# gsalzer/mythril

Hardware: AMD Instinct MI355X
Metric: constraint-candidate evals/sec + % z3 queries discharged on-GPU (higher is better)
Workload: dtype u32 (256-bit as 8x32-bit limbs)

## Files before the change

mythril_amd/csrc/u256.h:

```cpp
#pragma once
#include <math.h>
#include <stdint.h>

#define PF_INL __device__ __forceinline__

#include "u256_cols.h"

namespace pf {

struct u256 {
    uint32_t l[8];
};

PF_INL u256 zero256() {
    u256 r;
#pragma unroll
    for (int i = 0; i < 8; i++) r.l[i] = 0;
    return r;
}

PF_INL u256 ones256() {
    u256 r;
#pragma unroll
    for (int i = 0; i < 8; i++) r.l[i] = 0xffffffffu;
    return r;
}

PF_INL u256 add256(const u256& a, const u256& b) {
    u256 r;
    uint32_t c = 0;
#pragma unroll
    for (int i = 0; i < 8; i++) {
        uint32_t co;
        r.l[i] = __builtin_addc(a.l[i], b.l[i], c, &co);
        c = co;
    }
    return r;
}

PF_INL u256 add256c(const u256& a, const u256& b, uint32_t* cout) {
    u256 r;
    uint32_t c = 0;
#pragma unroll
    for (int i = 0; i < 8; i++) {
        uint32_t co;
        r.l[i] = __builtin_addc(a.l[i], b.l[i], c, &co);
        c = co;
    }
    *cout = c;
    return r;
}

PF_INL u256 sub256(const u256& a, const u256& b) {
    u256 r;
    uint32_t c = 0;
#pragma unroll
    for (int i = 0; i < 8; i++) {
        uint32_t co;
        r.l[i] = __builtin_subc(a.l[i], b.l[i], c, &co);
        c = co;
    }
    return r;
}

PF_INL u256 sub256b(const u256& a, const u256& b, uint32_t* bout) {
    u256 r;
    uint32_t c = 0;
#pragma unroll
    for (int i = 0; i < 8; i++) {
        uint32_t co;
        r.l[i] = __builtin_subc(a.l[i], b.l[i], c, &co);
        c = co;
    }
    *bout = c;
    return r;
}

PF_INL uint32_t ult256(const u256& a, const u256& b) {
    uint32_t c = 0;
#pragma unroll
    for (int i = 0; i < 8; i++) {
        uint32_t co;
        (void)__builtin_subc(a.l[i], b.l[i], c, &co);
        c = co;
    }
    return c;
}

PF_INL uint32_t eq256(const u256& a, const u256& b) {
    uint32_t d = 0;
#pragma unroll
    for (int i = 0; i < 8; i++) d |= a.l[i] ^ b.l[i];
    return d == 0;
}

PF_INL uint32_t iszero256(const u256& a) {
    uint32_t d = 0;
#pragma unroll
    for (int i = 0; i < 8; i++) d |= a.l[i];
    return d == 0;
}

PF_INL u256 neg256(const u256& a) { return sub256(zero256(), a); }

PF_INL u256 not256(const u256& a) {
    u256 r;
#pragma unroll
    for (int i = 0; i < 8; i++) r.l[i] = ~a.l[i];
    return r;
}

PF_INL uint32_t lane_mask(uint32_t c) {
    uint32_t m = 0u - (uint32_t)(c != 0u);
#ifndef PF_HOST_MAC
    asm volatile("" : "+v"(m));
#endif
    return m;
}

PF_INL u256 sel256(uint32_t c, const u256& a, const u256& b) {
    const uint32_t m = lane_mask(c);
    u256 r;
#pragma unroll
    for (int i = 0; i < 8; i++) r.l[i] = (a.l[i] & m) | (b.l[i] & ~m);
    return r;
}

#ifndef PF_HOST_MAC
PF_INL uint32_t wave_max_u32(uint32_t v) {
#pragma unroll
    for (int o = 32; o >= 1; o >>= 1) v = max(v, (uint32_t)__shfl_xor((int)v, o));
    return __builtin_amdgcn_readfirstlane(v);
}
PF_INL bool wave_any(bool p) { return __ballot(p) != 0ull; }
PF_INL uint32_t umulhi32(uint32_t a, uint32_t b) { return __umulhi(a, b); }
#else
PF_INL uint32_t wave_max_u32(uint32_t v) { return v; }
PF_INL bool wave_any(bool p) { return p; }
PF_INL uint32_t umulhi32(uint32_t a, uint32_t b) { return (uint32_t)(((uint64_t)a * b) >> 32); }
#endif

#define PF_COL_NEXT(k)                                   \
    r.l[k] = (uint32_t)acc;                              \
    acc = (acc >> 32) | ((uint64_t)hi << 32);            \
    hi = 0u;

PF_INL u256 mul256(const u256& a, const u256& b) {
    const uint32_t *x = a.l, *y = b.l;
    u256 r;
    uint64_t acc = 0;
    uint32_t hi = 0;
    col64_1(acc, x[0], y[0]);
    PF_COL_NEXT(0)
    col96_2(acc, hi, x[0], x[1], y[1], y[0]);
    PF_COL_NEXT(1)
    col96_3(acc, hi, x[0], x[1], x[2], y[2], y[1], y[0]);
    PF_COL_NEXT(2)
    col96_4(acc, hi, x[0], x[1], x[2], x[3], y[3], y[2], y[1], y[0]);
    PF_COL_NEXT(3)
    col96_5(acc, hi, x[0], x[1], x[2], x[3], x[4], y[4], y[3], y[2], y[1], y[0]);
    PF_COL_NEXT(4)
    col96_6(acc, hi, x[0], x[1], x[2], x[3], x[4], x[5], y[5], y[4], y[3], y[2], y[1], y[0]);
    PF_COL_NEXT(5)
    col64_7(acc, x[0], x[1], x[2], x[3], x[4], x[5], x[6], y[6], y[5], y[4], y[3], y[2], y[1], y[0]);
    r.l[6] = (uint32_t)acc;
    acc >>= 32;
    col64_8(acc, x[0], x[1], x[2], x[3], x[4], x[5], x[6], x[7], y[7], y[6], y[5], y[4], y[3], y[2], y[1], y[0]);
    r.l[7] = (uint32_t)acc;
    return r;
}

PF_INL u256 sqr256(const u256& a) {
    const uint32_t* x = a.l;
    u256 r;
    r.l[0] = 0u;
    uint64_t acc = 0;
    uint32_t hi = 0;
    col64_1(acc, x[0], x[1]);
    PF_COL_NEXT(1)
    col96_1(acc, hi, x[0], x[2]);
    PF_COL_NEXT(2)
    col96_2(acc, hi, x[0], x[1], x[3], x[2]);
    PF_COL_NEXT(3)
    col96_2(acc, hi, x[0], x[1], x[4], x[3]);
    PF_COL_NEXT(4)
    col96_3(acc, hi, x[0], x[1], x[2], x[5], x[4], x[3]);
    PF_COL_NEXT(5)
    col64_3(acc, x[0], x[1], x[2], x[6], x[5], x[4]);
    r.l[6] = (uint32_t)acc;
    acc >>= 32;
    col64_4(acc, x[0], x[1], x[2], x[3], x[7], x[6], x[5], x[4]);
    r.l[7] = (uint32_t)acc;
    u256 c;
#pragma unroll
    for (int i = 7; i >= 1; i--) c.l[i] = (r.l[i] << 1) | (r.l[i - 1] >> 31);
    c.l[0] = 0u;
    u256 d;
#pragma unroll
    for (int i = 0; i < 4; i++) {
        uint64_t q = 0;
        col64_1(q, x[i], x[i]);
        d.l[2 * i] = (uint32_t)q;
        d.l[2 * i + 1] = (uint32_t)(q >> 32);
    }
    return add256(c, d);
}
#undef PF_COL_NEXT

PF_INL uint32_t mul256_overflows(const u256& a, const u256& b) {
    uint32_t hi = 0;
    u256 r = zero256();
#pragma unroll
    for (int i = 0; i < 8; i++) {
        uint64_t carry = 0;
#pragma unroll
        for (int j = 0; j < 8; j++) {
            if (i + j < 8) {
                uint64_t t = (uint64_t)a.l[i] * b.l[j] + r.l[i + j] + carry;
                r.l[i + j] = (uint32_t)t;
                carry = t >> 32;
            } else {
                hi |= (a.l[i] != 0u && b.l[j] != 0u) ? 1u : 0u;
            }
        }
        hi |= (carry != 0) ? 1u : 0u;
    }
    return hi;
}

PF_INL u256 shl256(const u256& a, uint32_t s, uint32_t big) {
    u256 x = a;
    if (__builtin_expect(1, 1)) {
        uint32_t m = (s >> 7) & 1;
#pragma unroll
        for (int i = 7; i >= 0; i--) x.l[i] = m ? (i >= 4 ? x.l[i - 4] : 0u) : x.l[i];
        m = (s >> 6) & 1;
#pragma unroll
        for (int i = 7; i >= 0; i--) x.l[i] = m ? (i >= 2 ? x.l[i - 2] : 0u) : x.l[i];
        m = (s >> 5) & 1;
#pragma unroll
        for (int i = 7; i >= 0; i--) x.l[i] = m ? (i >= 1 ? x.l[i - 1] : 0u) : x.l[i];
    }
    uint32_t bs = s & 31;
    u256 r;
#pragma unroll
    for (int i = 7; i >= 1; i--) r.l[i] = bs ? ((x.l[i] << bs) | (x.l[i - 1] >> (32 - bs))) : x.l[i];
    r.l[0] = x.l[0] << bs;
    return sel256(big, zero256(), r);
}

PF_INL u256 shr256(const u256& a, uint32_t s, uint32_t f) {
    u256 x = a;
    uint32_t m = (s >> 7) & 1;
#pragma unroll
    for (int i = 0; i < 8; i++) x.l[i] = m ? (i + 4 < 8 ? x.l[i + 4] : f) : x.l[i];
    m = (s >> 6) & 1;
#pragma unroll
    for (int i = 0; i < 8; i++) x.l[i] = m ? (i + 2 < 8 ? x.l[i + 2] : f) : x.l[i];
    m = (s >> 5) & 1;
#pragma unroll
    for (int i = 0; i < 8; i++) x.l[i] = m ? (i + 1 < 8 ? x.l[i + 1] : f) : x.l[i];
    uint32_t bs = s & 31;
    u256 r;
#pragma unroll
    for (int i = 0; i < 7; i++) r.l[i] = bs ? ((x.l[i] >> bs) | (x.l[i + 1] << (32 - bs))) : x.l[i];
    r.l[7] = bs ? ((x.l[7] >> bs) | (f << (32 - bs))) : x.l[7];
    return r;
}

PF_INL uint32_t clz256(const u256& a) {
    uint32_t n = 0, done = 0;
#pragma unroll
    for (int i = 7; i >= 0; i--) {
        uint32_t z = a.l[i] ? (uint32_t)__builtin_clz(a.l[i]) : 32u;
        n += done ? 0u : z;
        done |= (a.l[i] != 0u);
    }
    return n;
}

PF_INL double rcp_f64(double x) {
#ifndef PF_HOST_MAC
    double r = __builtin_amdgcn_rcp(x);
    double e = fma(-x, r, 1.0);
    r = fma(r, e, r);
    e = fma(-x, r, 1.0);
    return fma(r, e, r);
#else
    return 1.0 / x;
#endif
}

// ... 94 lines not shown
#pragma unroll
        for (int i = 0; i + j <= 8; i++) {
            const uint64_t p = (uint64_t)q * (i < 8 ? b.l[i] : 0u) + carry;
            carry = p >> 32;
            uint32_t bo;
            u[j + i] = __builtin_subc(u[j + i], (uint32_t)p, borrow, &bo);
            borrow = bo;
        }
        if (wave_any(borrow != 0u)) {
            const uint32_t m = 0u - borrow;
            q -= borrow;
            uint32_t c = 0;
#pragma unroll
            for (int i = 0; i + j <= 8; i++) {
                uint32_t co;
                u[j + i] = __builtin_addc(u[j + i], (i < 8 ? b.l[i] : 0u) & m, c, &co);
                c = co;
            }
        }
        Q.l[j] = q;
    }
    u256 R;
#pragma unroll
    for (int i = 0; i < 8; i++) R.l[i] = u[i];
    *q = sel256(bz, ones256(), Q);
    *r = sel256(bz, a, R);
}

PF_INL void tbl_put(uint2* tbl, uint32_t stride, uint32_t j, const u256& v) {
#pragma unroll
    for (int p = 0; p < 4; p++) tbl[(j * 4u + p) * stride] = make_uint2(v.l[2 * p], v.l[2 * p + 1]);
}
PF_INL u256 tbl_get(const uint2* tbl, uint32_t stride, uint32_t j) {
    u256 v;
#pragma unroll
    for (int p = 0; p < 4; p++) {
        const uint2 q = tbl[(j * 4u + p) * stride];
        v.l[2 * p] = q.x;
        v.l[2 * p + 1] = q.y;
    }
    return v;
}

template <int WB = 3>
PF_INL u256 exp256(const u256& base, const u256& e, uint32_t nbits, uint2* tbl, uint32_t stride) {
    static_assert(WB >= 1 && WB <= 3, "window");
    constexpr uint32_t NT = 1u << WB;
    u256 r = zero256();
    r.l[0] = 1u;
    if (nbits == 0u) return r;
    tbl_put(tbl, stride, 0u, r);
    tbl_put(tbl, stride, 1u, base);
    if constexpr (WB == 2) {
        const u256 b2 = sqr256(base);
        tbl_put(tbl, stride, 2u, b2);
        tbl_put(tbl, stride, 3u, mul256(b2, base));
    } else {
#pragma unroll 1
        for (uint32_t j = 2; j < NT; j++) {
            const u256 f = tbl_get(tbl, stride, (j & 1u) ? j - 1u : j >> 1);
            const u256 g = (j & 1u) ? base : f;
            tbl_put(tbl, stride, j, mul256(f, g));
        }
    }
    const uint32_t nd = (nbits + WB - 1u) / WB;
    const uint32_t rest = WB * (nd - 1u);
    r = tbl_get(tbl, stride, shr256(e, rest, 0u).l[0] & (NT - 1u));
    u256 ex = shl256(e, (256u - rest) & 255u, 0u);
#pragma unroll 1
    for (uint32_t i = 1; i < nd; i++) {
#pragma unroll 1
        for (int k = 0; k < WB; k++) r = sqr256(r);
        const uint32_t d = ex.l[7] >> (32 - WB);
#pragma unroll
        for (int k = 7; k >= 1; k--) ex.l[k] = (ex.l[k] << WB) | (ex.l[k - 1] >> (32 - WB));
        ex.l[0] <<= WB;
        r = mul256(r, tbl_get(tbl, stride, d));
    }
    return r;
}

template <int WB = 2>
PF_INL u256 exp256_w32(const u256& base, uint32_t e, uint32_t nbits, uint2* tbl, uint32_t stride) {
    static_assert(WB == 2, "window");
    u256 one = zero256();
    one.l[0] = 1u;
    tbl_put(tbl, stride, 1u, base);
    const u256 b2 = sqr256(base);
    tbl_put(tbl, stride, 2u, b2);
    tbl_put(tbl, stride, 3u, mul256(b2, base));
    if (nbits == 0u) return one;
    const uint32_t nd = (nbits + WB - 1u) / WB;
    uint32_t d = (e >> (WB * (nd - 1u))) & 3u;
    u256 r = sel256((uint32_t)(d == 0u), one, tbl_get(tbl, stride, d));
#pragma unroll 1
    for (uint32_t i = nd - 1u; i-- > 0u;) {
#pragma unroll 1
        for (int k = 0; k < WB; k++) r = sqr256(r);
        d = (e >> (WB * i)) & 3u;
        r = mul256(r, sel256((uint32_t)(d == 0u), one, tbl_get(tbl, stride, d)));
    }
    return r;
}

#ifndef PF_EXP_SPLIT
#define PF_EXP_SPLIT 8
#endif
#define PF_EXP_WINDOW (PF_EXP_SPLIT <= 20 ? 2 : 3)
#define PF_EXP_TBL_ENTRIES (1 << PF_EXP_WINDOW)

PF_INL uint32_t funnel(uint32_t hi, uint32_t lo, uint32_t s) {
    return (uint32_t)((((uint64_t)hi << 32) | lo) >> s);
}

template <int L>
PF_INL void tsqr(const uint32_t* a, uint32_t* out) {
    uint32_t r[L];
#pragma unroll
    for (int i = 0; i < L; i++) r[i] = 0u;
#pragma unroll
    for (int i = 0; 2 * i + 1 < L; i++) {
        uint64_t c = 0;
#pragma unroll
        for (int j = i + 1; i + j < L; j++) {
            c = (uint64_t)a[i] * a[j] + (uint64_t)r[i + j] + (c >> 32);
            r[i + j] = (uint32_t)c;
        }
    }
#pragma unroll
    for (int i = L - 1; i >= 1; i--) r[i] = funnel(r[i], r[i - 1], 31u);
    r[0] <<= 1;
    uint32_t d[L];
#pragma unroll
    for (int i = 0; 2 * i < L; i++) {
        const uint64_t q = (uint64_t)a[i] * a[i];
        d[2 * i] = (uint32_t)q;
        if (2 * i + 1 < L) d[2 * i + 1] = (uint32_t)(q >> 32);
    }
    uint32_t c = 0;
#pragma unroll
    for (int i = 0; i < L; i++) {
        uint32_t co;
        out[i] = __builtin_addc(r[i], d[i], c, &co);
        c = co;
    }
}

template <int TL, uint32_t TM, int Q>
PF_INL void t_steps(uint32_t* t, uint32_t k0, uint32_t k1) {
    constexpr int L = TL - Q;
#pragma unroll 1
    for (uint32_t k = k0; k < k1; k++) {
        uint32_t sq[L];
        tsqr<L>(t, sq);
        const uint32_t sh = 32u - (k + 1u - 32u * Q);
        uint32_t c = 0;
#pragma unroll
        for (int i = Q; i < TL; i++) {
            const uint32_t lo = i > Q ? sq[i > Q ? i - Q - 1 : 0] : 0u;
            uint32_t co;
            t[i] = __builtin_addc(t[i], funnel(sq[i - Q], lo, sh), c, &co);
            c = co;
        }
        t[TL - 1] &= TM;
    }
}


PF_INL u256 div_odd_small(const u256& a, uint32_t o, uint32_t inv) {
    u256 q;
    uint32_t s = 0;
#pragma unroll
    for (int i = 0; i < 8; i++) {
        const uint32_t ai = a.l[i] - s;
        const uint32_t bo = a.l[i] < s;
        q.l[i] = ai * inv;
        s = umulhi32(q.l[i], o) + bo;
    }
    return q;
}

constexpr int v2c(int i) { return (i & 1) ? 0 : 1 + v2c(i >> 1); }
constexpr int v2fact(int j) { return j <= 1 ? 0 : v2c(j) + v2fact(j - 1); }
constexpr int exp_terms(int m) {
    int j = 1;
    while ((j + 1) * (m + 2) - v2fact(j + 1) < 256) j++;
    return j;
}
constexpr uint32_t inv32(uint32_t o) {
    uint32_t x = o;
    for (int i = 0; i < 5; i++) x *= 2u - o * x;
    return x;
}
constexpr int prefix_val(int m, int i) { return (i - 1) * (m + 2) - v2fact(i - 1); }

template <int L>
PF_INL u256 tmul(const u256& a, const u256& b) {
    if constexpr (L >= 8) {
        return mul256(a, b);
    } else {
        u256 r = zero256();
#pragma unroll
        for (int i = 0; i < L; i++) {
            uint64_t c = 0;
#pragma unroll
            for (int j = 0; i + j < L; j++) {
                c = (uint64_t)a.l[i] * b.l[j] + (uint64_t)r.l[i + j] + (c >> 32);
                r.l[i + j] = (uint32_t)c;
            }
        }
        return r;
    }
}

template <int L>
PF_INL u256 sub_mul_small(const u256& a, const u256& b, uint32_t c) {
    u256 r = zero256();
    uint32_t carry = 0, bw = 0;
#pragma unroll
    for (int i = 0; i < L; i++) {
        const uint64_t p = (uint64_t)b.l[i] * c + carry;
        carry = (uint32_t)(p >> 32);
        uint32_t bo;
        r.l[i] = __builtin_subc(a.l[i], (uint32_t)p, bw, &bo);
        bw = bo;
    }
    return r;
}

template <int L>
PF_INL u256 div_odd_small(const u256& a, uint32_t o, uint32_t inv) {
    u256 q = zero256();
    uint32_t s = 0;
#pragma unroll
    for (int i = 0; i < L; i++) {
        const uint32_t ai = a.l[i] - s;
        const uint32_t bo = a.l[i] < s;
        q.l[i] = ai * inv;
        s = umulhi32(q.l[i], o) + bo;
    }
    return q;
}

template <int S, int L>
PF_INL u256 shl_const(const u256& a) {
    constexpr int LS = S / 32, BS = S % 32;
    u256 r = zero256();
#pragma unroll
    for (int i = LS; i < L; i++) {
        const uint32_t hi = a.l[i - LS];
        const uint32_t lo = i - LS - 1 >= 0 ? a.l[i - LS - 1 >= 0 ? i - LS - 1 : 0] : 0u;
        r.l[i] = BS ? funnel(hi, lo, 32 - BS) : hi;
    }
    return r;
}

template <int M, int I, int J>
PF_INL u256 horner(const u256& nt, const u256& tt) {
    constexpr int S = M + 2 - v2c(I);
    constexpr int P = 256 - prefix_val(M, I);
    constexpr int L = (P + 31) / 32;
    constexpr int LG = (P - S + 31) / 32;
    constexpr int O = I >> v2c(I);
    u256 inner = zero256();
    if constexpr (I < J) inner = horner<M, I + 1, J>(nt, tt);
    u256 g = I > 1 ? sub_mul_small<LG>(nt, tt, (uint32_t)(I - 1)) : nt;
    if (O > 1) g = div_odd_small<LG>(g, (uint32_t)O, inv32((uint32_t)O));
    u256 h = shl_const<S, L>(g);
    if constexpr (I < J) h = tmul<L>(h, inner);
    h.l[0] += 1u;
    return h;
}

PF_INL u256 exp256_split(const u256& base, const u256& e, uint2* tbl, uint32_t stride,
                         uint64_t* pt = nullptr) {
#if defined(PF_PROFILE_UNITS) && !defined(PF_HOST_MAC)
#define PF_EXP_STAMP(k)                                        \
    if (pt) {                                                  \
        const uint64_t t_ = __builtin_amdgcn_s_memtime();      \
        pt[k] += t_ - t_last;                                  \
        t_last = t_;                                           \
    }
    uint64_t t_last = __builtin_amdgcn_s_memtime();
#else
#define PF_EXP_STAMP(k)
    (void)pt;
#endif
    constexpr int M = PF_EXP_SPLIT;
    static_assert(M >= 8 && M <= 84, "split");
    constexpr int T = 254 - M;
    constexpr int TL = (T + 31) / 32;
    constexpr uint32_t TM = (T % 32) ? ((1u << (T % 32)) - 1u) : 0xffffffffu;
    constexpr int TB = (T + 3 + 31) / 32;
    constexpr int J = exp_terms(M);
    constexpr int WB = PF_EXP_WINDOW;
    const uint32_t odd = base.l[0] & 1u;
    const uint32_t e_big =
        (e.l[0] >= 256u) | ((e.l[1] | e.l[2] | e.l[3] | e.l[4] | e.l[5] | e.l[6] | e.l[7]) != 0u);
    u256 e0;
#pragma unroll
    for (int i = 0; i < 8; i++)
        e0.l[i] = 32 * i + 32 <= M ? e.l[i] : (32 * i < M ? e.l[i] & ((1u << (M % 32)) - 1u) : 0u);
    const uint32_t nb0 = wave_max_u32(256u - clz256(e0));
    u256 r;
    if constexpr (M <= 32 && WB == 2)
        r = exp256_w32<WB>(base, e0.l[0], nb0 < (uint32_t)M ? nb0 : (uint32_t)M, tbl, stride);
    else
        r = exp256<WB>(base, e0, nb0 < (uint32_t)M ? nb0 : (uint32_t)M, tbl, stride);
    PF_EXP_STAMP(0)
    u256 n = shr256(e, (uint32_t)M, 0u);
#pragma unroll
    for (int i = 0; i < 8; i++) n.l[i] = i < TL - 1 ? n.l[i] : (i == TL - 1 ? n.l[i] & TM : 0u);
    if (wave_any(odd & (iszero256(n) ^ 1u))) {
        tbl_put(tbl, stride, 1u, r);
        uint32_t t[TL];
        {
            uint32_t sq[TB];
            if constexpr (M <= 32 && WB == 2 && TB == 8) {
                const u256 b2 = tbl_get(tbl, stride, 2u);
#pragma unroll
                for (int i = 0; i < TB; i++) sq[i] = b2.l[i];
            } else {
                tsqr<TB>(base.l, sq);
            }
            sq[0] -= 1u;
#pragma unroll
            for (int i = 0; i < TL; i++) t[i] = funnel(i + 1 < TB ? sq[i + 1 < TB ? i + 1 : 0] : 0u, sq[i], 3u);
            t[TL - 1] &= TM;
        }
        t_steps<TL, TM, 0>(t, 1u, M < 32 ? (uint32_t)M : 32u);
        if (M > 32) t_steps<TL, TM, 1>(t, 32u, M < 64 ? (uint32_t)M : 64u);
        if (M > 64) t_steps<TL, TM, 2>(t, 64u, (uint32_t)M);
        u256 tt = zero256();
#pragma unroll
        for (int i = 0; i < TL; i++) tt.l[i] = t[i];
        PF_EXP_STAMP(1)
        const u256 nt = tmul<(256 - (M + 2) + 31) / 32>(n, tt);
        u256 h = horner<M, 1, J>(nt, tt);
        u256 one = zero256();
        one.l[0] = 1u;
        h = sel256(odd, h, one);
        r = mul256(tbl_get(tbl, stride, 1u), h);
        PF_EXP_STAMP(2)
    }
    return sel256((odd ^ 1u) & e_big, zero256(), r);
#undef PF_EXP_STAMP
}

}
```

mythril_amd/csrc/u256_cols.h:

```cpp
#pragma once
namespace pf {
#ifndef PF_HOST_MAC

PF_INL void col96_1(uint64_t& acc, uint32_t& hi, uint32_t x0, uint32_t y0) {
    uint64_t p0;
    asm("v_mad_u64_u32 %[acc], %[p0], %[x0], %[y0], %[acc]\n\ts_nop 1\n\tv_addc_co_u32_e64 %[hi], %[p0], %[hi], 0, %[p0]"
        : [acc] "+v"(acc), [hi] "+v"(hi), [p0] "=&s"(p0)
        : [x0] "v"(x0), [y0] "v"(y0));
}

PF_INL void col96_2(uint64_t& acc, uint32_t& hi, uint32_t x0, uint32_t x1, uint32_t y0, uint32_t y1) {
    uint64_t p0; uint64_t p1;
    asm("v_mad_u64_u32 %[acc], %[p0], %[x0], %[y0], %[acc]\n\tv_mad_u64_u32 %[acc], %[p1], %[x1], %[y1], %[acc]\n\ts_nop 0\n\tv_addc_co_u32_e64 %[hi], %[p0], %[hi], 0, %[p0]\n\tv_addc_co_u32_e64 %[hi], %[p1], %[hi], 0, %[p1]"
        : [acc] "+v"(acc), [hi] "+v"(hi), [p0] "=&s"(p0), [p1] "=&s"(p1)
        : [x0] "v"(x0), [x1] "v"(x1), [y0] "v"(y0), [y1] "v"(y1));
}

PF_INL void col96_3(uint64_t& acc, uint32_t& hi, uint32_t x0, uint32_t x1, uint32_t x2, uint32_t y0, uint32_t y1, uint32_t y2) {
    uint64_t p0; uint64_t p1; uint64_t p2;
    asm("v_mad_u64_u32 %[acc], %[p0], %[x0], %[y0], %[acc]\n\tv_mad_u64_u32 %[acc], %[p1], %[x1], %[y1], %[acc]\n\tv_mad_u64_u32 %[acc], %[p2], %[x2], %[y2], %[acc]\n\tv_addc_co_u32_e64 %[hi], %[p0], %[hi], 0, %[p0]\n\tv_addc_co_u32_e64 %[hi], %[p1], %[hi], 0, %[p1]\n\tv_addc_co_u32_e64 %[hi], %[p2], %[hi], 0, %[p2]"
        : [acc] "+v"(acc), [hi] "+v"(hi), [p0] "=&s"(p0), [p1] "=&s"(p1), [p2] "=&s"(p2)
        : [x0] "v"(x0), [x1] "v"(x1), [x2] "v"(x2), [y0] "v"(y0), [y1] "v"(y1), [y2] "v"(y2));
}

// ... 26 lines not shown
}

PF_INL void col64_2(uint64_t& acc, uint32_t x0, uint32_t x1, uint32_t y0, uint32_t y1) {
    uint64_t p;
    asm("v_mad_u64_u32 %[acc], %[p], %[x0], %[y0], %[acc]\n\tv_mad_u64_u32 %[acc], %[p], %[x1], %[y1], %[acc]"
        : [acc] "+v"(acc), [p] "=&s"(p)
        : [x0] "v"(x0), [x1] "v"(x1), [y0] "v"(y0), [y1] "v"(y1));
}

PF_INL void col64_3(uint64_t& acc, uint32_t x0, uint32_t x1, uint32_t x2, uint32_t y0, uint32_t y1, uint32_t y2) {
    uint64_t p;
    asm("v_mad_u64_u32 %[acc], %[p], %[x0], %[y0], %[acc]\n\tv_mad_u64_u32 %[acc], %[p], %[x1], %[y1], %[acc]\n\tv_mad_u64_u32 %[acc], %[p], %[x2], %[y2], %[acc]"
        : [acc] "+v"(acc), [p] "=&s"(p)
        : [x0] "v"(x0), [x1] "v"(x1), [x2] "v"(x2), [y0] "v"(y0), [y1] "v"(y1), [y2] "v"(y2));
}

PF_INL void col64_4(uint64_t& acc, uint32_t x0, uint32_t x1, uint32_t x2, uint32_t x3, uint32_t y0, uint32_t y1, uint32_t y2, uint32_t y3) {
    uint64_t p;
    asm("v_mad_u64_u32 %[acc], %[p], %[x0], %[y0], %[acc]\n\tv_mad_u64_u32 %[acc], %[p], %[x1], %[y1], %[acc]\n\tv_mad_u64_u32 %[acc], %[p], %[x2], %[y2], %[acc]\n\tv_mad_u64_u32 %[acc], %[p], %[x3], %[y3], %[acc]"
        : [acc] "+v"(acc), [p] "=&s"(p)
        : [x0] "v"(x0), [x1] "v"(x1), [x2] "v"(x2), [x3] "v"(x3), [y0] "v"(y0), [y1] "v"(y1), [y2] "v"(y2), [y3] "v"(y3));
}

PF_INL void col64_5(uint64_t& acc, uint32_t x0, uint32_t x1, uint32_t x2, uint32_t x3, uint32_t x4, uint32_t y0, uint32_t y1, uint32_t y2, uint32_t y3, uint32_t y4) {
    uint64_t p;
    asm("v_mad_u64_u32 %[acc], %[p], %[x0], %[y0], %[acc]\n\tv_mad_u64_u32 %[acc], %[p], %[x1], %[y1], %[acc]\n\tv_mad_u64_u32 %[acc], %[p], %[x2], %[y2], %[acc]\n\tv_mad_u64_u32 %[acc], %[p], %[x3], %[y3], %[acc]\n\tv_mad_u64_u32 %[acc], %[p], %[x4], %[y4], %[acc]"
        : [acc] "+v"(acc), [p] "=&s"(p)
        : [x0] "v"(x0), [x1] "v"(x1), [x2] "v"(x2), [x3] "v"(x3), [x4] "v"(x4), [y0] "v"(y0), [y1] "v"(y1), [y2] "v"(y2), [y3] "v"(y3), [y4] "v"(y4));
}

PF_INL void col64_6(uint64_t& acc, uint32_t x0, uint32_t x1, uint32_t x2, uint32_t x3, uint32_t x4, uint32_t x5, uint32_t y0, uint32_t y1, uint32_t y2, uint32_t y3, uint32_t y4, uint32_t y5) {
    uint64_t p;
    asm("v_mad_u64_u32 %[acc], %[p], %[x0], %[y0], %[acc]\n\tv_mad_u64_u32 %[acc], %[p], %[x1], %[y1], %[acc]\n\tv_mad_u64_u32 %[acc], %[p], %[x2], %[y2], %[acc]\n\tv_mad_u64_u32 %[acc], %[p], %[x3], %[y3], %[acc]\n\tv_mad_u64_u32 %[acc], %[p], %[x4], %[y4], %[acc]\n\tv_mad_u64_u32 %[acc], %[p], %[x5], %[y5], %[acc]"
        : [acc] "+v"(acc), [p] "=&s"(p)
        : [x0] "v"(x0), [x1] "v"(x1), [x2] "v"(x2), [x3] "v"(x3), [x4] "v"(x4), [x5] "v"(x5), [y0] "v"(y0), [y1] "v"(y1), [y2] "v"(y2), [y3] "v"(y3), [y4] "v"(y4), [y5] "v"(y5));
}

PF_INL void col64_7(uint64_t& acc, uint32_t x0, uint32_t x1, uint32_t x2, uint32_t x3, uint32_t x4, uint32_t x5, uint32_t x6, uint32_t y0, uint32_t y1, uint32_t y2, uint32_t y3, uint32_t y4, uint32_t y5, uint32_t y6) {
    uint64_t p;
    asm("v_mad_u64_u32 %[acc], %[p], %[x0], %[y0], %[acc]\n\tv_mad_u64_u32 %[acc], %[p], %[x1], %[y1], %[acc]\n\tv_mad_u64_u32 %[acc], %[p], %[x2], %[y2], %[acc]\n\tv_mad_u64_u32 %[acc], %[p], %[x3], %[y3], %[acc]\n\tv_mad_u64_u32 %[acc], %[p], %[x4], %[y4], %[acc]\n\tv_mad_u64_u32 %[acc], %[p], %[x5], %[y5], %[acc]\n\tv_mad_u64_u32 %[acc], %[p], %[x6], %[y6], %[acc]"
        : [acc] "+v"(acc), [p] "=&s"(p)
        : [x0] "v"(x0), [x1] "v"(x1), [x2] "v"(x2), [x3] "v"(x3), [x4] "v"(x4), [x5] "v"(x5), [x6] "v"(x6), [y0] "v"(y0), [y1] "v"(y1), [y2] "v"(y2), [y3] "v"(y3), [y4] "v"(y4), [y5] "v"(y5), [y6] "v"(y6));
}

PF_INL void col64_8(uint64_t& acc, uint32_t x0, uint32_t x1, uint32_t x2, uint32_t x3, uint32_t x4, uint32_t x5, uint32_t x6, uint32_t x7, uint32_t y0, uint32_t y1, uint32_t y2, uint32_t y3, uint32_t y4, uint32_t y5, uint32_t y6, uint32_t y7) {
    uint64_t p;
    asm("v_mad_u64_u32 %[acc], %[p], %[x0], %[y0], %[acc]\n\tv_mad_u64_u32 %[acc], %[p], %[x1], %[y1], %[acc]\n\tv_mad_u64_u32 %[acc], %[p], %[x2], %[y2], %[acc]\n\tv_mad_u64_u32 %[acc], %[p], %[x3], %[y3], %[acc]\n\tv_mad_u64_u32 %[acc], %[p], %[x4], %[y4], %[acc]\n\tv_mad_u64_u32 %[acc], %[p], %[x5], %[y5], %[acc]\n\tv_mad_u64_u32 %[acc], %[p], %[x6], %[y6], %[acc]\n\tv_mad_u64_u32 %[acc], %[p], %[x7], %[y7], %[acc]"
        : [acc] "+v"(acc), [p] "=&s"(p)
        : [x0] "v"(x0), [x1] "v"(x1), [x2] "v"(x2), [x3] "v"(x3), [x4] "v"(x4), [x5] "v"(x5), [x6] "v"(x6), [x7] "v"(x7), [y0] "v"(y0), [y1] "v"(y1), [y2] "v"(y2), [y3] "v"(y3), [y4] "v"(y4), [y5] "v"(y5), [y6] "v"(y6), [y7] "v"(y7));
}

#else

PF_INL void col96_1(uint64_t& acc, uint32_t& hi, uint32_t x0, uint32_t y0) {
    { unsigned __int128 t = (unsigned __int128)x0 * y0 + acc; acc = (uint64_t)t; hi += (uint32_t)(t >> 64); }
}

PF_INL void col96_2(uint64_t& acc, uint32_t& hi, uint32_t x0, uint32_t x1, uint32_t y0, uint32_t y1) {
    { unsigned __int128 t = (unsigned __int128)x0 * y0 + acc; acc = (uint64_t)t; hi += (uint32_t)(t >> 64); }
    { unsigned __int128 t = (unsigned __int128)x1 * y1 + acc; acc = (uint64_t)t; hi += (uint32_t)(t >> 64); }
}

PF_INL void col96_3(uint64_t& acc, uint32_t& hi, uint32_t x0, uint32_t x1, uint32_t x2, uint32_t y0, uint32_t y1, uint32_t y2) {
    { unsigned __int128 t = (unsigned __int128)x0 * y0 + acc; acc = (uint64_t)t; hi += (uint32_t)(t >> 64); }
    { unsigned __int128 t = (unsigned __int128)x1 * y1 + acc; acc = (uint64_t)t; hi += (uint32_t)(t >> 64); }
    { unsigned __int128 t = (unsigned __int128)x2 * y2 + acc; acc = (uint64_t)t; hi += (uint32_t)(t >> 64); }
}

PF_INL void col96_4(uint64_t& acc, uint32_t& hi, uint32_t x0, uint32_t x1, uint32_t x2, uint32_t x3, uint32_t y0, uint32_t y1, uint32_t y2, uint32_t y3) {
    { unsigned __int128 t = (unsigned __int128)x0 * y0 + acc; acc = (uint64_t)t; hi += (uint32_t)(t >> 64); }
    { unsigned __int128 t = (unsigned __int128)x1 * y1 + acc; acc = (uint64_t)t; hi += (uint32_t)(t >> 64); }
    { unsigned __int128 t = (unsigned __int128)x2 * y2 + acc; acc = (uint64_t)t; hi += (uint32_t)(t >> 64); }
    { unsigned __int128 t = (unsigned __int128)x3 * y3 + acc; acc = (uint64_t)t; hi += (uint32_t)(t >> 64); }
}

PF_INL void col96_5(uint64_t& acc, uint32_t& hi, uint32_t x0, uint32_t x1, uint32_t x2, uint32_t x3, uint32_t x4, uint32_t y0, uint32_t y1, uint32_t y2, uint32_t y3, uint32_t y4) {
    { unsigned __int128 t = (unsigned __int128)x0 * y0 + acc; acc = (uint64_t)t; hi += (uint32_t)(t >> 64); }
    { unsigned __int128 t = (unsigned __int128)x1 * y1 + acc; acc = (uint64_t)t; hi += (uint32_t)(t >> 64); }
    { unsigned __int128 t = (unsigned __int128)x2 * y2 + acc; acc = (uint64_t)t; hi += (uint32_t)(t >> 64); }
    { unsigned __int128 t = (unsigned __int128)x3 * y3 + acc; acc = (uint64_t)t; hi += (uint32_t)(t >> 64); }
    { unsigned __int128 t = (unsigned __int128)x4 * y4 + acc; acc = (uint64_t)t; hi += (uint32_t)(t >> 64); }
}

PF_INL void col96_6(uint64_t& acc, uint32_t& hi, uint32_t x0, uint32_t x1, uint32_t x2, uint32_t x3, uint32_t x4, uint32_t x5, uint32_t y0, uint32_t y1, uint32_t y2, uint32_t y3, uint32_t y4, uint32_t y5) {
    { unsigned __int128 t = (unsigned __int128)x0 * y0 + acc; acc = (uint64_t)t; hi += (uint32_t)(t >> 64); }
    { unsigned __int128 t = (unsigned __int128)x1 * y1 + acc; acc = (uint64_t)t; hi += (uint32_t)(t >> 64); }
    { unsigned __int128 t = (unsigned __int128)x2 * y2 + acc; acc = (uint64_t)t; hi += (uint32_t)(t >> 64); }
    { unsigned __int128 t = (unsigned __int128)x3 * y3 + acc; acc = (uint64_t)t; hi += (uint32_t)(t >> 64); }
    { unsigned __int128 t = (unsigned __int128)x4 * y4 + acc; acc = (uint64_t)t; hi += (uint32_t)(t >> 64); }
    { unsigned __int128 t = (unsigned __int128)x5 * y5 + acc; acc = (uint64_t)t; hi += (uint32_t)(t >> 64); }
}

PF_INL void col64_1(uint64_t& acc, uint32_t x0, uint32_t y0) {
    acc += (uint64_t)x0 * y0;
}

PF_INL void col64_2(uint64_t& acc, uint32_t x0, uint32_t x1, uint32_t y0, uint32_t y1) {
    acc += (uint64_t)x0 * y0;
    acc += (uint64_t)x1 * y1;
}

PF_INL void col64_3(uint64_t& acc, uint32_t x0, uint32_t x1, uint32_t x2, uint32_t y0, uint32_t y1, uint32_t y2) {
    acc += (uint64_t)x0 * y0;
    acc += (uint64_t)x1 * y1;
    acc += (uint64_t)x2 * y2;
}

PF_INL void col64_4(uint64_t& acc, uint32_t x0, uint32_t x1, uint32_t x2, uint32_t x3, uint32_t y0, uint32_t y1, uint32_t y2, uint32_t y3) {
    acc += (uint64_t)x0 * y0;
    acc += (uint64_t)x1 * y1;
    acc += (uint64_t)x2 * y2;
    acc += (uint64_t)x3 * y3;
}

PF_INL void col64_5(uint64_t& acc, uint32_t x0, uint32_t x1, uint32_t x2, uint32_t x3, uint32_t x4, uint32_t y0, uint32_t y1, uint32_t y2, uint32_t y3, uint32_t y4) {
    acc += (uint64_t)x0 * y0;
    acc += (uint64_t)x1 * y1;
    acc += (uint64_t)x2 * y2;
    acc += (uint64_t)x3 * y3;
    acc += (uint64_t)x4 * y4;
}

PF_INL void col64_6(uint64_t& acc, uint32_t x0, uint32_t x1, uint32_t x2, uint32_t x3, uint32_t x4, uint32_t x5, uint32_t y0, uint32_t y1, uint32_t y2, uint32_t y3, uint32_t y4, uint32_t y5) {
    acc += (uint64_t)x0 * y0;
    acc += (uint64_t)x1 * y1;
    acc += (uint64_t)x2 * y2;
    acc += (uint64_t)x3 * y3;
    acc += (uint64_t)x4 * y4;
    acc += (uint64_t)x5 * y5;
}

PF_INL void col64_7(uint64_t& acc, uint32_t x0, uint32_t x1, uint32_t x2, uint32_t x3, uint32_t x4, uint32_t x5, uint32_t x6, uint32_t y0, uint32_t y1, uint32_t y2, uint32_t y3, uint32_t y4, uint32_t y5, uint32_t y6) {
    acc += (uint64_t)x0 * y0;
    acc += (uint64_t)x1 * y1;
    acc += (uint64_t)x2 * y2;
    acc += (uint64_t)x3 * y3;
    acc += (uint64_t)x4 * y4;
    acc += (uint64_t)x5 * y5;
    acc += (uint64_t)x6 * y6;
}

PF_INL void col64_8(uint64_t& acc, uint32_t x0, uint32_t x1, uint32_t x2, uint32_t x3, uint32_t x4, uint32_t x5, uint32_t x6, uint32_t x7, uint32_t y0, uint32_t y1, uint32_t y2, uint32_t y3, uint32_t y4, uint32_t y5, uint32_t y6, uint32_t y7) {
    acc += (uint64_t)x0 * y0;
    acc += (uint64_t)x1 * y1;
    acc += (uint64_t)x2 * y2;
    acc += (uint64_t)x3 * y3;
    acc += (uint64_t)x4 * y4;
    acc += (uint64_t)x5 * y5;
    acc += (uint64_t)x6 * y6;
    acc += (uint64_t)x7 * y7;
}

#endif
}
```

Baseline: 6.786 billion.

## Reformulate exp Horner with precomputed constant addends, drop per-term odd divisions

```diff
diff --git a/mythril_amd/csrc/u256.h b/mythril_amd/csrc/u256.h
--- a/mythril_amd/csrc/u256.h
+++ b/mythril_amd/csrc/u256.h
@@ -133,11 +133,9 @@
     return __builtin_amdgcn_readfirstlane(v);
 }
 PF_INL bool wave_any(bool p) { return __ballot(p) != 0ull; }
-PF_INL uint32_t umulhi32(uint32_t a, uint32_t b) { return __umulhi(a, b); }
 #else
 PF_INL uint32_t wave_max_u32(uint32_t v) { return v; }
 PF_INL bool wave_any(bool p) { return p; }
-PF_INL uint32_t umulhi32(uint32_t a, uint32_t b) { return (uint32_t)(((uint64_t)a * b) >> 32); }
 #endif
 
 #define PF_COL_NEXT(k)                                   \
@@ -538,7 +536,16 @@
 #pragma unroll 1
     for (uint32_t k = k0; k < k1; k++) {
         uint32_t sq[L];
-        tsqr<L>(t, sq);
+        if constexpr (L == 8) {
+            u256 a;
+#pragma unroll
+            for (int i = 0; i < 8; i++) a.l[i] = t[i];
+            const u256 s = sqr256(a);
+#pragma unroll
+            for (int i = 0; i < 8; i++) sq[i] = s.l[i];
+        } else {
+            tsqr<L>(t, sq);
+        }
         const uint32_t sh = 32u - (k + 1u - 32u * Q);
         uint32_t c = 0;
 #pragma unroll
@@ -552,19 +559,6 @@
     }
 }
 
-
-PF_INL u256 div_odd_small(const u256& a, uint32_t o, uint32_t inv) {
-    u256 q;
-    uint32_t s = 0;
-#pragma unroll
-    for (int i = 0; i < 8; i++) {
-        const uint32_t ai = a.l[i] - s;
-        const uint32_t bo = a.l[i] < s;
-        q.l[i] = ai * inv;
-        s = umulhi32(q.l[i], o) + bo;
-    }
-    return q;
-}
 
 constexpr int v2c(int i) { return (i & 1) ? 0 : 1 + v2c(i >> 1); }
 constexpr int v2fact(int j) { return j <= 1 ? 0 : v2c(j) + v2fact(j - 1); }
@@ -573,30 +567,73 @@
     while ((j + 1) * (m + 2) - v2fact(j + 1) < 256) j++;
     return j;
 }
-constexpr uint32_t inv32(uint32_t o) {
-    uint32_t x = o;
-    for (int i = 0; i < 5; i++) x *= 2u - o * x;
+constexpr int prefix_val(int m, int i) { return (i - 1) * (m + 2) - v2fact(i - 1); }
+
+struct k256 {
+    uint32_t l[8];
+};
+constexpr k256 k_small(uint32_t v) {
+    k256 r{};
+    r.l[0] = v;
+    return r;
+}
+constexpr k256 k_mul(const k256& a, const k256& b) {
+    k256 r{};
+    for (int i = 0; i < 8; i++) {
+        uint64_t c = 0;
+        for (int j = 0; i + j < 8; j++) {
+            c = (uint64_t)a.l[i] * b.l[j] + r.l[i + j] + (c >> 32);
+            r.l[i + j] = (uint32_t)c;
+        }
+    }
+    return r;
+}
+constexpr k256 k_inv(const k256& o) {
+    k256 x = o;
+    for (int it = 0; it < 7; it++) {
+        const k256 ox = k_mul(o, x);
+        k256 two_minus{};
+        uint64_t bw = 0;
+        for (int i = 0; i < 8; i++) {
+            const uint64_t d = (uint64_t)(i == 0 ? 2u : 0u) - ox.l[i] - bw;
+            two_minus.l[i] = (uint32_t)d;
+            bw = (d >> 32) & 1u;
+        }
+        x = k_mul(x, two_minus);
+    }
     return x;
 }
-constexpr int prefix_val(int m, int i) { return (i - 1) * (m + 2) - v2fact(i - 1); }
+constexpr k256 exp_oddprod(int i, int j) {
+    k256 r = k_small(1u);
+    for (int k = i; k <= j; k++) r = k_mul(r, k_small((uint32_t)(k >> v2c(k))));
+    return r;
+}
+constexpr k256 exp_addend(int i, int j, int limbs) {
+    k256 r = k_mul(exp_oddprod(i, j), k_inv(exp_oddprod(1, j)));
+    for (int k = limbs; k < 8; k++) r.l[k] = 0u;
+    return r;
+}
+
+template <int L, int LY, uint32_t K0, uint32_t K1>
+PF_INL u256 tmul_add(const u256& a, const u256& b, const k256& k) {
+    if constexpr (L >= 8) {
+        u256 kk;
+#pragma unroll
+        for (int i = 0; i < 8; i++) kk.l[i] = k.l[i];
+        return add256(mul256(a, b), kk);
+    } else {
+        u256 r = zero256();
+        tmulk<L, LY, K0, K1>(a.l, b.l, k.l, r.l);
+        return r;
+    }
+}
 
 template <int L>
 PF_INL u256 tmul(const u256& a, const u256& b) {
-    if constexpr (L >= 8) {
+    if constexpr (L >= 8)
         return mul256(a, b);
-    } else {
-        u256 r = zero256();
-#pragma unroll
-        for (int i = 0; i < L; i++) {
-            uint64_t c = 0;
-#pragma unroll
-            for (int j = 0; i + j < L; j++) {
-                c = (uint64_t)a.l[i] * b.l[j] + (uint64_t)r.l[i + j] + (c >> 32);
-                r.l[i + j] = (uint32_t)c;
-            }
-        }
-        return r;
-    }
+    else
+        return tmul_add<L, L, 0u, 0u>(a, b, k256{});
 }
 
 template <int L>
@@ -614,20 +651,6 @@
     return r;
 }
 
-template <int L>
-PF_INL u256 div_odd_small(const u256& a, uint32_t o, uint32_t inv) {
-    u256 q = zero256();
-    uint32_t s = 0;
-#pragma unroll
-    for (int i = 0; i < L; i++) {
-        const uint32_t ai = a.l[i] - s;
-        const uint32_t bo = a.l[i] < s;
-        q.l[i] = ai * inv;
-        s = umulhi32(q.l[i], o) + bo;
-    }
-    return q;
-}
-
 template <int S, int L>
 PF_INL u256 shl_const(const u256& a) {
     constexpr int LS = S / 32, BS = S % 32;
@@ -642,20 +665,22 @@
 }
 
 template <int M, int I, int J>
-PF_INL u256 horner(const u256& nt, const u256& tt) {
+PF_INL u256 horner(u256& g, const u256& tt) {
     constexpr int S = M + 2 - v2c(I);
     constexpr int P = 256 - prefix_val(M, I);
     constexpr int L = (P + 31) / 32;
-    constexpr int LG = (P - S + 31) / 32;
-    constexpr int O = I >> v2c(I);
+    constexpr k256 K = exp_addend(I, J, L);
+    constexpr int LY = (I == J || (P - S + 31) / 32 >= L || L == 1) ? L : L - 1;
     u256 inner = zero256();
-    if constexpr (I < J) inner = horner<M, I + 1, J>(nt, tt);
-    u256 g = I > 1 ? sub_mul_small<LG>(nt, tt, (uint32_t)(I - 1)) : nt;
-    if (O > 1) g = div_odd_small<LG>(g, (uint32_t)O, inv32((uint32_t)O));
-    u256 h = shl_const<S, L>(g);
-    if constexpr (I < J) h = tmul<L>(h, inner);
-    h.l[0] += 1u;
-    return h;
+    if constexpr (I < J) {
+        inner = horner<M, I + 1, J>(g, tt);
+        g = add256(g, tt);
+    } else {
+        constexpr k256 C = exp_addend(J + 1, J, L);
+#pragma unroll
+        for (int i = 0; i < L; i++) inner.l[i] = C.l[i];
+    }
+    return tmul_add<L, LY, K.l[0], K.l[1]>(shl_const<S, L>(g), inner, K);
 }
 
 PF_INL u256 exp256_split(const u256& base, const u256& e, uint2* tbl, uint32_t stride,
@@ -722,7 +747,8 @@
         for (int i = 0; i < TL; i++) tt.l[i] = t[i];
         PF_EXP_STAMP(1)
         const u256 nt = tmul<(256 - (M + 2) + 31) / 32>(n, tt);
-        u256 h = horner<M, 1, J>(nt, tt);
+        u256 g = sub_mul_small<8>(nt, tt, (uint32_t)(J - 1));
+        u256 h = horner<M, 1, J>(g, tt);
         u256 one = zero256();
         one.l[0] = 1u;
         h = sel256(odd, h, one);
diff --git a/mythril_amd/csrc/u256_cols.h b/mythril_amd/csrc/u256_cols.h
--- a/mythril_amd/csrc/u256_cols.h
+++ b/mythril_amd/csrc/u256_cols.h
@@ -202,4 +202,278 @@
 }
 
 #endif
-}
+
+template <uint32_t K0, uint32_t K1>
+PF_INL uint64_t acc_const() {
+#ifndef PF_HOST_MAC
+    if constexpr (K0 != 0u || K1 != 0u) {
+        uint32_t lo, up;
+        asm volatile("v_mov_b32 %0, %2\n\tv_mov_b32 %1, %3" : "=v"(lo), "=v"(up) : "i"(K0), "i"(K1));
+        return (uint64_t)lo | ((uint64_t)up << 32);
+    }
+#endif
+    return (uint64_t)K0 | ((uint64_t)K1 << 32);
+}
+
+template <uint32_t K0, uint32_t K1>
+PF_INL void tmulk_1_1(const uint32_t* x, const uint32_t* y, const uint32_t* k, uint32_t* r) {
+    uint64_t acc = acc_const<K0, 0u>();
+    uint32_t hi = 0u;
+    col64_1(acc, x[0], y[0]);
+    r[0] = (uint32_t)acc;
+    (void)hi;
+}
+
+template <uint32_t K0, uint32_t K1>
+PF_INL void tmulk_2_1(const uint32_t* x, const uint32_t* y, const uint32_t* k, uint32_t* r) {
+    uint64_t acc = acc_const<K0, K1>();
+    uint32_t hi = 0u;
+    col64_1(acc, x[0], y[0]);
+    r[0] = (uint32_t)acc;
+    acc >>= 32;
+    col64_1(acc, x[1], y[0]);
+    r[1] = (uint32_t)acc;
+    (void)hi;
+}
+
+template <uint32_t K0, uint32_t K1>
+PF_INL void tmulk_2_2(const uint32_t* x, const uint32_t* y, const uint32_t* k, uint32_t* r) {
+    uint64_t acc = acc_const<K0, K1>();
+    uint32_t hi = 0u;
+    col64_1(acc, x[0], y[0]);
+    r[0] = (uint32_t)acc;
+    acc >>= 32;
+    col64_2(acc, x[0], x[1], y[1], y[0]);
+    r[1] = (uint32_t)acc;
+    (void)hi;
+}
+
+template <uint32_t K0, uint32_t K1>
+PF_INL void tmulk_3_2(const uint32_t* x, const uint32_t* y, const uint32_t* k, uint32_t* r) {
+    uint64_t acc = acc_const<K0, K1>();
+    uint32_t hi = 0u;
+    col96_1(acc, hi, x[0], y[0]);
+    r[0] = (uint32_t)acc;
+    { const uint64_t t = (uint64_t)hi + k[2]; acc = (acc >> 32) | (t << 32); hi = (uint32_t)(t >> 32); }
+    col64_2(acc, x[0], x[1], y[1], y[0]);
+    r[1] = (uint32_t)acc;
+    acc >>= 32;
+    col64_2(acc, x[1], x[2], y[1], y[0]);
+    r[2] = (uint32_t)acc;
+    (void)hi;
+}
+
+template <uint32_t K0, uint32_t K1>
+PF_INL void tmulk_3_3(const uint32_t* x, const uint32_t* y, const uint32_t* k, uint32_t* r) {
+    uint64_t acc = acc_const<K0, K1>();
+    uint32_t hi = 0u;
+    col96_1(acc, hi, x[0], y[0]);
+    r[0] = (uint32_t)acc;
+    { const uint64_t t = (uint64_t)hi + k[2]; acc = (acc >> 32) | (t << 32); hi = (uint32_t)(t >> 32); }
+    col64_2(acc, x[0], x[1], y[1], y[0]);
+    r[1] = (uint32_t)acc;
+    acc >>= 32;
+    col64_3(acc, x[0], x[1], x[2], y[2], y[1], y[0]);
+    r[2] = (uint32_t)acc;
+    (void)hi;
+}
+
+template <uint32_t K0, uint32_t K1>
+PF_INL void tmulk_4_3(const uint32_t* x, const uint32_t* y, const uint32_t* k, uint32_t* r) {
+    uint64_t acc = acc_const<K0, K1>();
+    uint32_t hi = 0u;
+    col96_1(acc, hi, x[0], y[0]);
+    r[0] = (uint32_t)acc;
+    { const uint64_t t = (uint64_t)hi + k[2]; acc = (acc >> 32) | (t << 32); hi = (uint32_t)(t >> 32); }
+    col96_2(acc, hi, x[0], x[1], y[1], y[0]);
+    r[1] = (uint32_t)acc;
+    { const uint64_t t = (uint64_t)hi + k[3]; acc = (acc >> 32) | (t << 32); hi = (uint32_t)(t >> 32); }
+    col64_3(acc, x[0], x[1], x[2], y[2], y[1], y[0]);
+    r[2] = (uint32_t)acc;
+    acc >>= 32;
+    col64_3(acc, x[1], x[2], x[3], y[2], y[1], y[0]);
+    r[3] = (uint32_t)acc;
+    (void)hi;
+}
+
+template <uint32_t K0, uint32_t K1>
+PF_INL void tmulk_4_4(const uint32_t* x, const uint32_t* y, const uint32_t* k, uint32_t* r) {
+    uint64_t acc = acc_const<K0, K1>();
+    uint32_t hi = 0u;
+    col96_1(acc, hi, x[0], y[0]);
+    r[0] = (uint32_t)acc;
+    { const uint64_t t = (uint64_t)hi + k[2]; acc = (acc >> 32) | (t << 32); hi = (uint32_t)(t >> 32); }
+    col96_2(acc, hi, x[0], x[1], y[1], y[0]);
+    r[1] = (uint32_t)acc;
+    { const uint64_t t = (uint64_t)hi + k[3]; acc = (acc >> 32) | (t << 32); hi = (uint32_t)(t >> 32); }
+    col64_3(acc, x[0], x[1], x[2], y[2], y[1], y[0]);
+    r[2] = (uint32_t)acc;
+    acc >>= 32;
+    col64_4(acc, x[0], x[1], x[2], x[3], y[3], y[2], y[1], y[0]);
+    r[3] = (uint32_t)acc;
+    (void)hi;
+}
+
+template <uint32_t K0, uint32_t K1>
+PF_INL void tmulk_5_4(const uint32_t* x, const uint32_t* y, const uint32_t* k, uint32_t* r) {
+    uint64_t acc = acc_const<K0, K1>();
+    uint32_t hi = 0u;
+    col96_1(acc, hi, x[0], y[0]);
+    r[0] = (uint32_t)acc;
+    { const uint64_t t = (uint64_t)hi + k[2]; acc = (acc >> 32) | (t << 32); hi = (uint32_t)(t >> 32); }
+    col96_2(acc, hi, x[0], x[1], y[1], y[0]);
+    r[1] = (uint32_t)acc;
+    { const uint64_t t = (uint64_t)hi + k[3]; acc = (acc >> 32) | (t << 32); hi = (uint32_t)(t >> 32); }
+    col96_3(acc, hi, x[0], x[1], x[2], y[2], y[1], y[0]);
+    r[2] = (uint32_t)acc;
+    { const uint64_t t = (uint64_t)hi + k[4]; acc = (acc >> 32) | (t << 32); hi = (uint32_t)(t >> 32); }
+    col64_4(acc, x[0], x[1], x[2], x[3], y[3], y[2], y[1], y[0]);
+    r[3] = (uint32_t)acc;
+    acc >>= 32;
+    col64_4(acc, x[1], x[2], x[3], x[4], y[3], y[2], y[1], y[0]);
+    r[4] = (uint32_t)acc;
+    (void)hi;
+}
+
+template <uint32_t K0, uint32_t K1>
+PF_INL void tmulk_5_5(const uint32_t* x, const uint32_t* y, const uint32_t* k, uint32_t* r) {
+    uint64_t acc = acc_const<K0, K1>();
+    uint32_t hi = 0u;
+    col96_1(acc, hi, x[0], y[0]);
+    r[0] = (uint32_t)acc;
+    { const uint64_t t = (uint64_t)hi + k[2]; acc = (acc >> 32) | (t << 32); hi = (uint32_t)(t >> 32); }
+    col96_2(acc, hi, x[0], x[1], y[1], y[0]);
+    r[1] = (uint32_t)acc;
+    { const uint64_t t = (uint64_t)hi + k[3]; acc = (acc >> 32) | (t << 32); hi = (uint32_t)(t >> 32); }
+    col96_3(acc, hi, x[0], x[1], x[2], y[2], y[1], y[0]);
+    r[2] = (uint32_t)acc;
+    { const uint64_t t = (uint64_t)hi + k[4]; acc = (acc >> 32) | (t << 32); hi = (uint32_t)(t >> 32); }
+    col64_4(acc, x[0], x[1], x[2], x[3], y[3], y[2], y[1], y[0]);
+    r[3] = (uint32_t)acc;
+    acc >>= 32;
+    col64_5(acc, x[0], x[1], x[2], x[3], x[4], y[4], y[3], y[2], y[1], y[0]);
+    r[4] = (uint32_t)acc;
+    (void)hi;
+}
+
+template <uint32_t K0, uint32_t K1>
+PF_INL void tmulk_6_5(const uint32_t* x, const uint32_t* y, const uint32_t* k, uint32_t* r) {
+    uint64_t acc = acc_const<K0, K1>();
+    uint32_t hi = 0u;
+    col96_1(acc, hi, x[0], y[0]);
+    r[0] = (uint32_t)acc;
+    { const uint64_t t = (uint64_t)hi + k[2]; acc = (acc >> 32) | (t << 32); hi = (uint32_t)(t >> 32); }
+    col96_2(acc, hi, x[0], x[1], y[1], y[0]);
+    r[1] = (uint32_t)acc;
+    { const uint64_t t = (uint64_t)hi + k[3]; acc = (acc >> 32) | (t << 32); hi = (uint32_t)(t >> 32); }
+    col96_3(acc, hi, x[0], x[1], x[2], y[2], y[1], y[0]);
+    r[2] = (uint32_t)acc;
+    { const uint64_t t = (uint64_t)hi + k[4]; acc = (acc >> 32) | (t << 32); hi = (uint32_t)(t >> 32); }
+    col96_4(acc, hi, x[0], x[1], x[2], x[3], y[3], y[2], y[1], y[0]);
+    r[3] = (uint32_t)acc;
+    { const uint64_t t = (uint64_t)hi + k[5]; acc = (acc >> 32) | (t << 32); hi = (uint32_t)(t >> 32); }
+    col64_5(acc, x[0], x[1], x[2], x[3], x[4], y[4], y[3], y[2], y[1], y[0]);
+    r[4] = (uint32_t)acc;
+    acc >>= 32;
+    col64_5(acc, x[1], x[2], x[3], x[4], x[5], y[4], y[3], y[2], y[1], y[0]);
+    r[5] = (uint32_t)acc;
+    (void)hi;
+}
+
+template <uint32_t K0, uint32_t K1>
+PF_INL void tmulk_6_6(const uint32_t* x, const uint32_t* y, const uint32_t* k, uint32_t* r) {
+    uint64_t acc = acc_const<K0, K1>();
+    uint32_t hi = 0u;
+    col96_1(acc, hi, x[0], y[0]);
+    r[0] = (uint32_t)acc;
+    { const uint64_t t = (uint64_t)hi + k[2]; acc = (acc >> 32) | (t << 32); hi = (uint32_t)(t >> 32); }
+    col96_2(acc, hi, x[0], x[1], y[1], y[0]);
+    r[1] = (uint32_t)acc;
+    { const uint64_t t = (uint64_t)hi + k[3]; acc = (acc >> 32) | (t << 32); hi = (uint32_t)(t >> 32); }
+    col96_3(acc, hi, x[0], x[1], x[2], y[2], y[1], y[0]);
+    r[2] = (uint32_t)acc;
+    { const uint64_t t = (uint64_t)hi + k[4]; acc = (acc >> 32) | (t << 32); hi = (uint32_t)(t >> 32); }
+    col96_4(acc, hi, x[0], x[1], x[2], x[3], y[3], y[2], y[1], y[0]);
+    r[3] = (uint32_t)acc;
+    { const uint64_t t = (uint64_t)hi + k[5]; acc = (acc >> 32) | (t << 32); hi = (uint32_t)(t >> 32); }
+    col64_5(acc, x[0], x[1], x[2], x[3], x[4], y[4], y[3], y[2], y[1], y[0]);
+    r[4] = (uint32_t)acc;
+    acc >>= 32;
+    col64_6(acc, x[0], x[1], x[2], x[3], x[4], x[5], y[5], y[4], y[3], y[2], y[1], y[0]);
+    r[5] = (uint32_t)acc;
+    (void)hi;
+}
+
+template <uint32_t K0, uint32_t K1>
+PF_INL void tmulk_7_6(const uint32_t* x, const uint32_t* y, const uint32_t* k, uint32_t* r) {
+    uint64_t acc = acc_const<K0, K1>();
+    uint32_t hi = 0u;
+    col96_1(acc, hi, x[0], y[0]);
+    r[0] = (uint32_t)acc;
+    { const uint64_t t = (uint64_t)hi + k[2]; acc = (acc >> 32) | (t << 32); hi = (uint32_t)(t >> 32); }
+    col96_2(acc, hi, x[0], x[1], y[1], y[0]);
+    r[1] = (uint32_t)acc;
+    { const uint64_t t = (uint64_t)hi + k[3]; acc = (acc >> 32) | (t << 32); hi = (uint32_t)(t >> 32); }
+    col96_3(acc, hi, x[0], x[1], x[2], y[2], y[1], y[0]);
+    r[2] = (uint32_t)acc;
+    { const uint64_t t = (uint64_t)hi + k[4]; acc = (acc >> 32) | (t << 32); hi = (uint32_t)(t >> 32); }
+    col96_4(acc, hi, x[0], x[1], x[2], x[3], y[3], y[2], y[1], y[0]);
+    r[3] = (uint32_t)acc;
+    { const uint64_t t = (uint64_t)hi + k[5]; acc = (acc >> 32) | (t << 32); hi = (uint32_t)(t >> 32); }
+    col96_5(acc, hi, x[0], x[1], x[2], x[3], x[4], y[4], y[3], y[2], y[1], y[0]);
+    r[4] = (uint32_t)acc;
+    { const uint64_t t = (uint64_t)hi + k[6]; acc = (acc >> 32) | (t << 32); hi = (uint32_t)(t >> 32); }
+    col64_6(acc, x[0], x[1], x[2], x[3], x[4], x[5], y[5], y[4], y[3], y[2], y[1], y[0]);
+    r[5] = (uint32_t)acc;
+    acc >>= 32;
+    col64_6(acc, x[1], x[2], x[3], x[4], x[5], x[6], y[5], y[4], y[3], y[2], y[1], y[0]);
+    r[6] = (uint32_t)acc;
+    (void)hi;
+}
+
+template <uint32_t K0, uint32_t K1>
+PF_INL void tmulk_7_7(const uint32_t* x, const uint32_t* y, const uint32_t* k, uint32_t* r) {
+    uint64_t acc = acc_const<K0, K1>();
+    uint32_t hi = 0u;
+    col96_1(acc, hi, x[0], y[0]);
+    r[0] = (uint32_t)acc;
+    { const uint64_t t = (uint64_t)hi + k[2]; acc = (acc >> 32) | (t << 32); hi = (uint32_t)(t >> 32); }
+    col96_2(acc, hi, x[0], x[1], y[1], y[0]);
+    r[1] = (uint32_t)acc;
+    { const uint64_t t = (uint64_t)hi + k[3]; acc = (acc >> 32) | (t << 32); hi = (uint32_t)(t >> 32); }
+    col96_3(acc, hi, x[0], x[1], x[2], y[2], y[1], y[0]);
+    r[2] = (uint32_t)acc;
+    { const uint64_t t = (uint64_t)hi + k[4]; acc = (acc >> 32) | (t << 32); hi = (uint32_t)(t >> 32); }
+    col96_4(acc, hi, x[0], x[1], x[2], x[3], y[3], y[2], y[1], y[0]);
+    r[3] = (uint32_t)acc;
+    { const uint64_t t = (uint64_t)hi + k[5]; acc = (acc >> 32) | (t << 32); hi = (uint32_t)(t >> 32); }
+    col96_5(acc, hi, x[0], x[1], x[2], x[3], x[4], y[4], y[3], y[2], y[1], y[0]);
+    r[4] = (uint32_t)acc;
+    { const uint64_t t = (uint64_t)hi + k[6]; acc = (acc >> 32) | (t << 32); hi = (uint32_t)(t >> 32); }
+    col64_6(acc, x[0], x[1], x[2], x[3], x[4], x[5], y[5], y[4], y[3], y[2], y[1], y[0]);
+    r[5] = (uint32_t)acc;
+    acc >>= 32;
+    col64_7(acc, x[0], x[1], x[2], x[3], x[4], x[5], x[6], y[6], y[5], y[4], y[3], y[2], y[1], y[0]);
+    r[6] = (uint32_t)acc;
+    (void)hi;
+}
+
+template <int L, int LY, uint32_t K0, uint32_t K1>
+PF_INL void tmulk(const uint32_t* x, const uint32_t* y, const uint32_t* k, uint32_t* r) {
+    static_assert(L >= 1 && L <= 7 && (LY == L || LY == L - 1) && LY >= 1, "shape");
+    if constexpr (L == 1 && LY == 1) tmulk_1_1<K0, K1>(x, y, k, r);
+    if constexpr (L == 2 && LY == 1) tmulk_2_1<K0, K1>(x, y, k, r);
+    if constexpr (L == 2 && LY == 2) tmulk_2_2<K0, K1>(x, y, k, r);
+    if constexpr (L == 3 && LY == 2) tmulk_3_2<K0, K1>(x, y, k, r);
+    if constexpr (L == 3 && LY == 3) tmulk_3_3<K0, K1>(x, y, k, r);
+    if constexpr (L == 4 && LY == 3) tmulk_4_3<K0, K1>(x, y, k, r);
+    if constexpr (L == 4 && LY == 4) tmulk_4_4<K0, K1>(x, y, k, r);
+    if constexpr (L == 5 && LY == 4) tmulk_5_4<K0, K1>(x, y, k, r);
+    if constexpr (L == 5 && LY == 5) tmulk_5_5<K0, K1>(x, y, k, r);
+    if constexpr (L == 6 && LY == 5) tmulk_6_5<K0, K1>(x, y, k, r);
+    if constexpr (L == 6 && LY == 6) tmulk_6_6<K0, K1>(x, y, k, r);
+    if constexpr (L == 7 && LY == 6) tmulk_7_6<K0, K1>(x, y, k, r);
+    if constexpr (L == 7 && LY == 7) tmulk_7_7<K0, K1>(x, y, k, r);
+}
+
+}
```

Measured after the change: 7.045 billion, median of 6. +3.8%, better.
